# yahoo/bftkv

Measured on AMD Instinct MI355X. Metric: pgp_rsa2048_signature_verifies_per_sec, higher is better.
Workload: dtype u32; 1 GPU; 64-replica quorum, 10000 RSA-2048 signed writes per GPU (cfg2 of BASELINE.json), 534164 signature packets per GPU, 1.0% corrupt / 0.5% unknown issuer / 0.5% duplicate / 1.0% one-short; parallelism=shard-by-write x1, RCCL all-gather of verdict bitmaps on the verifier's stream, replicas=64, writes_per_gpu=10000, sigs_per_gpu=534164, batches_in_flight=3

## Files before the change

### bftkv_amd/csrc/capi.hip

```cpp
#include "../../include/bftkv_gpu.h"

#include <hip/hip_runtime.h>
#include <stdio.h>
#include <stdlib.h>
#include <string.h>

#include <limits.h>
#include <linux/futex.h>
#include <sched.h>
#include <sys/syscall.h>
#include <unistd.h>

#include <algorithm>
#include <array>
#include <atomic>
#include <memory>
#include <functional>
#include <map>
#include <set>
#include <chrono>
#include <condition_variable>
#include <mutex>
#include <shared_mutex>
#include <system_error>
// ... 28 lines not shown
  hipError_t ensure_exact(size_t bytes) {
    if (bytes <= cap) return hipSuccess;
    if (p) { hipError_t e = hipFree(p); if (e != hipSuccess) return e; p = nullptr; cap = 0; }
    hipError_t e = hipMalloc(&p, bytes);
    if (e == hipSuccess) cap = bytes;
    return e;
  }
  void release() { if (p) (void)hipFree(p); p = nullptr; cap = 0; }
  template <typename T> T* as() const { return (T*)p; }
};

struct KeyEntry {
  uint64_t key_id = 0, entity_id = 0;
  uint8_t algo = 0, flags = 0;
  uint32_t bits = 0, e = 0, n0 = 0, qbits = 0;
  std::vector<uint32_t> nl, r2, r2w, qw, dtab, qpow, qconst;
  std::string material;
  bool cert_only = false;
  int cert_group = -1;
  uint32_t entity_index = 0;
  std::string cert_digest;
  uint64_t last_used = 0;
  bool dsa_unslotted = false;
};

struct QuorumHost {
  bool live = false;
  int n_qcs = 0;
  int32_t f[MAX_QC], mn[MAX_QC], thr[MAX_QC], suff[MAX_QC];
  std::vector<std::vector<uint64_t>> nodes;
// ... 12 lines not shown
  hipStream_t stream = nullptr;
  hipStream_t stream_h = nullptr;
  hipStream_t stream_d = nullptr;
  std::recursive_mutex mu;
  std::string err;

  uint64_t keyring_gen = 0;
  uint32_t n_keys = 0, n_entities = 0;
  bool have_dsa_keys = false, have_rsa3072 = false, have_rsa4096 = false, have_ambiguous = false;
  std::vector<uint64_t> h_key_id, h_entity_id;
  std::vector<uint32_t> h_key_entity;
  std::vector<uint8_t> h_key_flags;
  std::vector<KeyEntry> ring, certs;
  uint32_t n_ring_entities = 0;
  std::map<std::string, bool> cert_valid;
  DevBuf k_r2w;
  DevBuf k_id, k_entity, k_algo, k_flags, k_bits, k_e, k_n, k_r2, k_n0, k_q, k_qbits, k_dsatab, k_dsaslot, k_sorted_id, k_sorted_slot;
  DevBuf dsa_comb;
  uint32_t dsa_wbits = 8, dsa_wbits_pinned = 0;
  std::map<std::string, uint32_t> dsa_comb_slot;
  std::set<std::string> dsa_cert_materials;
  uint64_t ring_epoch = 0, dsa_ring_epoch_seen = ~0ull;
  uint32_t dsa_wbits_want = 0;
  uint32_t dsa_entry_limbs = DSA_N_SMALL;
  size_t dsa_budget_bytes = 0;
  bool have_dsa3072 = false, have_dsa2048 = false;
  DevBuf dsa_idx;
  uint64_t cert_clock = 0;
  struct CertFast { uint64_t issuer_id; int group; uint64_t epoch; };
  std::shared_mutex cert_fast_mu;
  std::unordered_map<std::string, CertFast> cert_fast;
// ... 421 lines not shown
  if (total && !d_mid_in && plan_q && big && c->h_mail) {
    const auto t_spin = std::chrono::steady_clock::now();
    for (uint32_t it = 0;; ++it) {
      const uint32_t v = __atomic_load_n(&c->h_mail[3], __ATOMIC_ACQUIRE);
      if (v) { other_hashes = (v & 1u) != 0; break; }
      if ((it & 255u) == 255u && std::chrono::steady_clock::now() - t_spin > std::chrono::microseconds(300) + std::chrono::nanoseconds((uint64_t)total / 2)) break;
      __builtin_ia32_pause();
    }
  }
  if (total && !d_mid_in && other_hashes)
    hipLaunchKernelGGL(k_digest_other, dim3(std::min<uint32_t>((total + 255) / 256, DIGEST_OTHER_MAX_BLOCKS)), dim3(256), 0, s,
                       d_tbs, d_tbs_off, d_ss, c->mid.as<uint32_t>(), c->mid64.as<uint64_t>(), n_items, c->recs.as<SigRec>(), total,
                       c->digests.as<uint32_t>(), c->pk_count.as<uint32_t>() + 4, txt, n_recs_dev);
  const dim3 cg(((uint64_t)total * CMP_LANES + 255) / 256);
  auto launch_compare = [&](const uint32_t* start) {
    hipLaunchKernelGGL(k_rsa_compare, cg, dim3(256), 0, s, c->recs.as<SigRec>(), c->pk_list.as<uint32_t>(),
                       cnt_p, start, c->kt, c->r.as<uint32_t>(), c->digests.as<uint32_t>());
    if (c->have_rsa3072)
      hipLaunchKernelGGL(k_rsa_compare, cg, dim3(256), 0, s, c->recs.as<SigRec>(), c->pk_list3072.as<uint32_t>(),
                         cnt_p + 2, start + 2, c->kt, c->r3072.as<uint32_t>(), c->digests.as<uint32_t>());
    if (c->have_rsa4096)
      hipLaunchKernelGGL(k_rsa_compare, cg, dim3(256), 0, s, c->recs.as<SigRec>(), c->pk_list4096.as<uint32_t>(),
                         cnt_p + 3, start + 3, c->kt, c->r4096.as<uint32_t>(), c->digests.as<uint32_t>());
  };
  auto launch_dsa = [&](const uint32_t* start) {
    hipLaunchKernelGGL(k_dsa_mul, dim3((total + 63) / 64), dim3(64), 0, s, c->recs.as<SigRec>(), c->dsa_list.as<uint32_t>(),
                       cnt_p, start, c->kt, c->digests.as<uint32_t>(), c->dsa_u.as<uint32_t>());
    const uint32_t* idx_s = nullptr; const uint32_t* idx_b = nullptr; const uint32_t* cnt_cls = nullptr;
    if (c->have_dsa3072 && c->have_dsa2048) {
      uint32_t* cc = cnt_p + (start == start0 ? 20 : 22);
      uint32_t* is = c->dsa_idx.as<uint32_t>() + (start == start0 ? 0 : 2 * (size_t)total);
      hipLaunchKernelGGL(k_dsa_split, dim3((total + 255) / 256), dim3(256), 0, s, c->recs.as<SigRec>(), c->dsa_list.as<uint32_t>(), cnt_p, start, c->kt,
// ... 22 lines not shown
    pl.verdict = c->o_verdict.as<uint8_t>();
    hipLaunchKernelGGL(k_plan<2>, dim3((n_items + PLAN_ITEMS - 1) / PLAN_ITEMS), dim3(PLAN_BLOCK), 0, s, pl, c->kt, *plan_q);
    const uint32_t* const start1 = cnt_p + 8;
    if (c->have_dsa_keys) launch_dsa_inv(s, start1);
    launch_modexp(start1);
    launch_compare(start1);
    if (c->have_dsa_keys) launch_dsa(start1);
  }
  if (total && c->have_ambiguous && !d_msg_slot)
    hipLaunchKernelGGL(k_candidates, dim3((total + 63) / 64), dim3(64), 0, s, d_tbs, d_tbs_off, d_ss, d_mid_in ? d_mid_in : c->mid.as<uint32_t>(),
                       c->mid64.as<uint64_t>(), n_items, c->recs.as<SigRec>(), total, n_recs_dev, d_tbs_prefix, c->kt, d_cert_ent, d_sig_class, txt,
                       c->hash_mask.as<uint32_t>());
  HIPCHK(c, rec(3, s));
  HIPCHK(c, hipGetLastError());
  return 0;
}

int make_key_entry(bftkv_gpu_ctx* c, const bftkv_gpu_pubkey& k, bool cert_only, KeyEntry* out) {
  KeyEntry& e = *out;
  e.key_id = k.key_id; e.entity_id = k.entity_id; e.algo = k.pk_algo; e.cert_only = cert_only;
  e.material.clear();
  e.material.push_back((char)k.pk_algo);
  e.material.push_back((char)k.usable_sign);
  auto app = [&](const uint8_t* p, uint32_t l) {
    uint32_t z = 0;
    while (z < l && p[z] == 0) ++z;
    if (l > z) e.material.append((const char*)p + z, l - z);
    e.material.push_back('|');
  };
  app(k.n, k.n_len); app(k.e, k.e_len); app(k.g, k.g_len); app(k.y, k.y_len);
  e.flags = 0;
  if (k.usable_sign) e.flags |= KEYF_USABLE_SIGN;
  if (k.pk_algo != PK_RSA_ENCRYPT_ONLY && k.pk_algo != PK_ELGAMAL) e.flags |= KEYF_CAN_SIGN;
  if (k.key_id == k.entity_id) e.flags |= KEYF_PRIMARY;
  if (cert_only) e.flags |= KEYF_CERT_ONLY;
  e.bits = (uint32_t)hostbn::bit_length(k.n, k.n_len);
  e.e = 0; e.n0 = 0; e.qbits = 0;
  e.r2w.clear();
  e.nl.assign(MONT_NMAX, 0); e.r2.assign(MONT_NMAX, 0); e.qw.assign(8, 0); e.dtab.assign(2 * DSA_N_BIG, 0); e.qpow.clear(); e.qconst.clear();
  if (k.pk_algo == PK_RSA || k.pk_algo == PK_RSA_SIGN_ONLY) {
    if (hostbn::bit_length(k.e, k.e_len) > 32) return fail(c, BFTKV_E_UNSUPPORTED, "RSA public exponent wider than 32 bits");
    for (uint32_t j = 0; j < k.e_len; ++j) e.e = (e.e << 8) | k.e[j];
    const int nlimbs = e.bits <= 2048 ? MONT_N : (e.bits <= 3072 ? MONT_TPI_BIG * MONT_L3072 : MONT_TPI_BIG * MONT_L4096);
    if (e.bits > 4096) e.bits = 0xFFFFFFFFu;
    else if (!hostbn::mont_setup(k.n, k.n_len, nlimbs, e.nl.data(), e.r2.data(), &e.n0)) e.bits = 0xFFFFFFFFu;
    else if (e.bits <= 2048) {
      std::vector<uint32_t> nl80(80);
      uint32_t n0b = 0;
      e.r2w.assign(80, 0);
      (void)hostbn::mont_setup(k.n, k.n_len, 80, nl80.data(), e.r2w.data(), &n0b);
    }
  } else if (k.pk_algo == PK_DSA) {
    e.qbits = (uint32_t)hostbn::bit_length(k.e, k.e_len);
    const int NLp = e.bits <= 2048 ? (int)DSA_N_SMALL : (int)DSA_N_BIG;
    const uint32_t cap_bits = e.bits <= 2048 ? 2048u : 3072u;
    const int nwords = (28 * NLp + 31) / 32 + 1;
    std::vector<uint32_t> p(nwords), g(nwords), y(nwords), q(nwords);
    hostbn::from_be(k.e, k.e_len, q.data(), nwords);
    bool ok = e.bits >= 2 && e.bits <= 3072 && e.qbits >= 32 && e.qbits <= 256 && (q[0] & 1u) &&
              hostbn::mont_setup(k.n, k.n_len, NLp, e.nl.data(), e.r2.data(), &e.n0);
    if (ok && (hostbn::bit_length(k.g, k.g_len) > cap_bits || hostbn::bit_length(k.y, k.y_len) > cap_bits)) ok = false;
    if (ok) {
      hostbn::from_be(k.n, k.n_len, p.data(), nwords);
      hostbn::from_be(k.g, k.g_len, g.data(), nwords);
      hostbn::from_be(k.y, k.y_len, y.data(), nwords);
// ... 187 lines not shown
                         (uint32_t)cs.size(), d_slots.as<uint32_t>(), d_rows.as<uint32_t>(), c->kt, c->dsa_comb.as<uint32_t>(), parts);
    else
      hipLaunchKernelGGL((k_dsa_build_comb<MONT_L, MONT_TPI>), dim3((n_groups + QUADS_PER_BLOCK - 1) / QUADS_PER_BLOCK), dim3(RSA_BLOCK), 0, c->stream,
                         (uint32_t)cs.size(), d_slots.as<uint32_t>(), d_rows.as<uint32_t>(), c->kt, c->dsa_comb.as<uint32_t>(), parts);
    e = hipStreamSynchronize(c->stream);
    d_slots.release(); d_rows.release();
  }
  if (e != hipSuccess) return fail(c, BFTKV_E_DEVICE, "k_dsa_build_comb", e);
  return 0;
}

int upload_key_table(bftkv_gpu_ctx* c) {
  if (c->root) return fail(c, BFTKV_E_STATE, "a forked context cannot change the key table (use its root)");
  KtWrite kw(c);
  std::vector<uint64_t> key_id, entity_ids;
  std::vector<uint32_t> entity, bits, e32, nl, r2, r2w, n0, qw, qbits, dtab;
  std::vector<uint8_t> algo, flags;
  std::vector<const KeyEntry*> rows;
  auto add = [&](const KeyEntry& e, bool own_entity) {
    uint32_t ent = 0;
    if (own_entity) { ent = (uint32_t)entity_ids.size(); entity_ids.push_back(e.entity_id); }
    else {
      for (; ent < entity_ids.size(); ++ent) if (entity_ids[ent] == e.entity_id) break;
      if (ent == entity_ids.size()) entity_ids.push_back(e.entity_id);
    }
    key_id.push_back(e.key_id); entity.push_back(ent); algo.push_back(e.algo); flags.push_back(e.flags);
    bits.push_back(e.bits); e32.push_back(e.e); n0.push_back(e.n0); qbits.push_back(e.qbits);
    nl.insert(nl.end(), e.nl.begin(), e.nl.end()); r2.insert(r2.end(), e.r2.begin(), e.r2.end());
    r2w.insert(r2w.end(), e.r2w.begin(), e.r2w.end()); r2w.resize(key_id.size() * 80, 0);
    qw.insert(qw.end(), e.qw.begin(), e.qw.end()); dtab.insert(dtab.end(), e.dtab.begin(), e.dtab.end());
    rows.push_back(&e);
    return ent;
  };
  for (auto& e : c->ring) add(e, false);
  c->n_ring_entities = (uint32_t)entity_ids.size();
  int last_group = -1;
  uint32_t group_ent = 0;
  std::vector<uint32_t> group_ents;
  for (auto& e : c->certs) {
    if (e.cert_group != last_group) { group_ent = add(e, true); last_group = e.cert_group; }
    else {
      key_id.push_back(e.key_id); entity.push_back(group_ent); algo.push_back(e.algo); flags.push_back(e.flags);
      bits.push_back(e.bits); e32.push_back(e.e); n0.push_back(e.n0); qbits.push_back(e.qbits);
      nl.insert(nl.end(), e.nl.begin(), e.nl.end()); r2.insert(r2.end(), e.r2.begin(), e.r2.end());
      r2w.insert(r2w.end(), e.r2w.begin(), e.r2w.end()); r2w.resize(key_id.size() * 80, 0);
      qw.insert(qw.end(), e.qw.begin(), e.qw.end()); dtab.insert(dtab.end(), e.dtab.begin(), e.dtab.end());
      rows.push_back(&e);
    }
    const_cast<KeyEntry&>(e).entity_index = group_ent;
    if (e.cert_group >= 0) {
      if (group_ents.size() <= (size_t)e.cert_group) group_ents.resize((size_t)e.cert_group + 1, 0xFFFFFFFEu);
      group_ents[(size_t)e.cert_group] = group_ent;
    }
  }
  std::vector<uint32_t> sorted_slot(key_id.size());
  for (size_t i = 0; i < sorted_slot.size(); ++i) sorted_slot[i] = (uint32_t)i;
  std::stable_sort(sorted_slot.begin(), sorted_slot.end(), [&](uint32_t a, uint32_t b) { return key_id[a] < key_id[b]; });
  std::vector<uint64_t> sorted_id(key_id.size());
  for (size_t i = 0; i < sorted_slot.size(); ++i) sorted_id[i] = key_id[sorted_slot[i]];
  int rc;
  if ((rc = upload(c, c->k_sorted_id, sorted_id)) || (rc = upload(c, c->k_sorted_slot, sorted_slot))) return rc;
  if ((rc = upload(c, c->k_id, key_id)) || (rc = upload(c, c->k_entity, entity)) || (rc = upload(c, c->k_algo, algo)) ||
      (rc = upload(c, c->k_flags, flags)) || (rc = upload(c, c->k_bits, bits)) || (rc = upload(c, c->k_e, e32)) ||
      (rc = upload(c, c->k_n, nl)) || (rc = upload(c, c->k_r2, r2)) || (rc = upload(c, c->k_n0, n0)) ||
      (rc = upload(c, c->k_q, qw)) || (rc = upload(c, c->k_qbits, qbits)) || (rc = upload(c, c->k_dsatab, dtab)) || (rc = upload(c, c->k_r2w, r2w)))
    return rc;
  c->kt.r2_limbs80 = c->k_r2w.as<uint32_t>();
  c->n_keys = (uint32_t)key_id.size();
  c->kt.n_keys = c->n_keys;
  c->kt.n_limbs = c->k_n.as<uint32_t>();
  c->kt.r2_limbs = c->k_r2.as<uint32_t>();
  c->kt.n0inv = c->k_n0.as<uint32_t>();
  c->kt.dsa_tab = c->k_dsatab.as<uint32_t>();
  bool bits_changed = false;
  if ((rc = sync_dsa_tables(c, rows, algo, bits, &bits_changed))) return rc;
  if (bits_changed && (rc = upload(c, c->k_bits, bits))) return rc;
  HIPCHK(c, hipStreamSynchronize(c->stream));
  c->have_dsa_keys = c->have_dsa3072 = c->have_dsa2048 = c->have_rsa3072 = c->have_rsa4096 = c->have_ambiguous = false;
  for (size_t i = 0; i < algo.size(); ++i) {
    if (flags[i] & KEYF_AMBIGUOUS) c->have_ambiguous = true;
    if (algo[i] == PK_DSA) c->have_dsa_keys = true;
    if (algo[i] == PK_DSA && bits[i] != 0xFFFFFFFFu && bits[i] > 2048) c->have_dsa3072 = true;
// ... 122 lines not shown
  if (!c) return;
  for (bftkv_gpu_ctx* w : c->hb_workers) bftkv_gpu_destroy(w);
  c->hb_workers.clear();
  if (!c->root && c->n_forks.load() > 0) {
    fprintf(stderr, "bftkv_gpu_destroy: context still has %d forked context(s); not destroyed\n", c->n_forks.load());
    return;
  }
  {
    std::lock_guard<std::mutex> lk(g_live_mu);
    for (size_t i = 0; i < g_live.size(); ++i) if (g_live[i] == c) { g_live.erase(g_live.begin() + i); break; }
  }
  (void)hipSetDevice(c->device);
  (void)hipStreamSynchronize(c->stream);
  (void)hipStreamSynchronize(c->stream_h);
  (void)hipStreamSynchronize(c->stream_d);
  for (DevBuf* b : {&c->k_id, &c->k_entity, &c->k_algo, &c->k_flags, &c->k_bits, &c->k_e, &c->k_n, &c->k_r2, &c->k_n0, &c->k_q, &c->k_qbits, &c->k_dsatab, &c->k_dsaslot, &c->dsa_comb, &c->k_sorted_id, &c->k_sorted_slot, &c->k_r2w,
                    &c->chunk_arena, &c->chunk_ctr, &c->counts, &c->base, &c->total, &c->item_flags, &c->walk_scratch, &c->cert_ent, &c->sig_class, &c->mid, &c->mid64, &c->hash_mask, &c->recs, &c->digests, &c->r, &c->xr,
                    &c->pk_list, &c->pk_list3072, &c->pk_list4096, &c->r3072, &c->r4096, &c->pk_count, &c->dsa_list, &c->dsa_u, &c->dsa_idx, &c->ids_tmp, &c->o_err, &c->o_nver, &c->o_verdict, &c->o_fenced, &c->in_tbs, &c->in_tbs_off,
                    &c->in_ss, &c->in_ss_off, &c->in_prefix, &c->in_prefix_off, &c->in_shared, &c->in_shared_off, &c->in_seg, &c->st_tmp, &c->item_tmp, &c->bits_tmp, &c->plan_cut, &c->txt_mid32, &c->txt_mid64, &c->txt_tail, &c->txt_len})
    b->release();
  for (auto& q : c->quorums) { q.member.release(); q.ids.release(); }
  c->in_pack.release();
  c->forced_iss.release();
  release_small_pin(c);
  if (c->h_out) (void)hipHostFree(c->h_out);
  if (c->root) c->root->n_forks.fetch_sub(1);
  for (DevBuf* b : c->scratch_pool) { b->release(); delete b; }
  for (auto& kv : c->modtab_cache) for (DevBuf& b : kv.second) b.release();
  for (DevBuf& b : c->ec_fb_tab) b.release();
  if (c->h_mail) (void)hipHostFree(c->h_mail);
  if (c->hb_out) (void)hipHostFree(c->hb_out);
// ... 953 lines not shown
```

### bftkv_amd/csrc/device_types.h

```cpp
#pragma once
#include <stdint.h>

namespace bftkv {

enum SigStatus : uint8_t {
  ST_OK = 0,
  ST_UNKNOWN_ISSUER = 1,
  ST_PARSE_ERROR = 2,
  ST_NOT_SIGNATURE = 3,
  ST_NO_ISSUER = 4,
  ST_HASH_UNSUPPORTED = 5,
  ST_HASH_TAG = 6,
  ST_ALGO_MISMATCH = 7,
  ST_BAD_SIG = 8,
  ST_KEY_CANNOT_SIGN = 9,
  ST_UNSUPPORTED = 10,
  ST_NOT_EXAMINED = 11,
  ST_PENDING_CHUNKED = 98,
  ST_PENDING_PARSE = 99,
  ST_PENDING_HASH = 100,
  ST_PENDING_RSA = 101,
  ST_PENDING_DSA = 102,
};

// ... 21 lines not shown

struct KeyTableDev {
  uint32_t n_keys;
  const uint64_t* key_id;
  const uint64_t* sorted_id;
  const uint32_t* sorted_slot;
  const uint32_t* entity;
  const uint8_t* pk_algo;
  const uint8_t* flags;
  const uint32_t* mod_bits;
  const uint32_t* rsa_e;
  const uint32_t* n_limbs;
  const uint32_t* r2_limbs;
  const uint32_t* r2_limbs80;
  const uint32_t* n0inv;
  const uint32_t* q_words;
  const uint32_t* q_bits;
  const uint32_t* dsa_tab;
  const uint32_t* dsa_slot;
  const uint32_t* dsa_comb;
  uint32_t dsa_wbits;
  uint32_t dsa_entry_limbs;
  uint32_t hash_policy;
};
constexpr uint32_t dsa_nwin(uint32_t wbits) { return (256u + wbits - 1u) / wbits; }
constexpr uint32_t DSA_N_SMALL = 76, DSA_N_BIG = 112;
constexpr uint64_t dsa_comb_limbs_per_key(uint32_t wbits, uint32_t entry_limbs) {
  return 2ull * dsa_nwin(wbits) * ((1u << wbits) - 1u) * entry_limbs;
}
constexpr uint32_t dsa_qpow_words(uint32_t entry_limbs) { return entry_limbs * 10u; }
constexpr uint32_t dsa_qtail_words(uint32_t entry_limbs) { return dsa_qpow_words(entry_limbs) + 12u; }
constexpr bool dsa_plain_window(uint32_t base, uint32_t w, uint32_t nwin) { return base == 1u && w == nwin - 1u; }
constexpr uint64_t dsa_slot_stride(uint32_t wbits, uint32_t entry_limbs) { return dsa_comb_limbs_per_key(wbits, entry_limbs) + dsa_qtail_words(entry_limbs); }

constexpr uint8_t KEYF_USABLE_SIGN = 1, KEYF_CAN_SIGN = 2, KEYF_PRIMARY = 4;
constexpr uint8_t KEYF_CERT_ONLY = 8;
constexpr uint8_t KEYF_CERT_CHECK_ONLY = 16;
constexpr uint8_t KEYF_AMBIGUOUS = 32;
constexpr uint32_t ITEM_FENCED = 0x80000000u;
constexpr uint32_t ITEM_TEXT_SHIFT = 8, ITEM_NEEDS_PAYLOAD = 0x7F7Eu;

struct TextDev {
  uint32_t* mid32;
  uint64_t* mid64;
  uint8_t* tail;
  uint64_t* len;
};

// ... 12 lines not shown
```

### bftkv_amd/csrc/host_bignum.h

```cpp
#pragma once
#include <stdint.h>
#include <string.h>

#include <vector>

namespace bftkv {
namespace hostbn {

constexpr int W28 = 28;
constexpr uint32_t MASK28 = (1u << W28) - 1;

inline void from_be(const uint8_t* be, uint32_t len, uint32_t* w, int nwords) {
  memset(w, 0, sizeof(uint32_t) * nwords);
  for (uint32_t i = 0; i < len; ++i) {
    uint32_t k = len - 1 - i;
    if ((int)(k >> 2) < nwords) w[k >> 2] |= (uint32_t)be[i] << (8 * (k & 3));
  }
}

inline int bit_length(const uint8_t* be, uint32_t len) {
  uint32_t i = 0;
  while (i < len && be[i] == 0) ++i;
  if (i == len) return 0;
  int top = 8;
// ... 120 lines not shown
  const uint32_t e = 2u * 28u * (uint32_t)nlimbs;
  int hb = 31;
  while (!((e >> hb) & 1u)) --hb;
  for (int b = hb - 1; b >= 0; --b) {
    montmul64(acc.data(), acc.data(), m.data(), m0inv, k, acc.data());
    if ((e >> b) & 1u) dbl_mod64(acc.data(), m.data(), k);
  }
  one[0] = 1;
  montmul64(acc.data(), one.data(), m.data(), m0inv, k, acc.data());
  std::vector<uint32_t> r(nwords, 0);
  for (int i = 0; i < nwords && i < 2 * k; ++i) r[i] = (uint32_t)(acc[i >> 1] >> (32 * (i & 1)));
  to_limbs28(r.data(), nwords, r2_limbs, nlimbs);
  return true;
}

inline void add_mod(uint32_t* a, const uint32_t* b, const uint32_t* m, int n) {
  uint64_t c = 0;
  for (int i = 0; i < n; ++i) { c += (uint64_t)a[i] + b[i]; a[i] = (uint32_t)c; c >>= 32; }
  if (c || cmp(a, m, n) >= 0) sub(a, m, n);
}
inline void mul_mod(const uint32_t* a, const uint32_t* b, const uint32_t* m, uint32_t* r, int n) {
  std::vector<uint32_t> acc(n, 0);
  for (int i = 32 * n - 1; i >= 0; --i) {
    dbl_mod(acc.data(), m, n);
    if ((b[i >> 5] >> (i & 31)) & 1u) add_mod(acc.data(), a, m, n);
  }
  memcpy(r, acc.data(), sizeof(uint32_t) * n);
}
inline void reduce(uint32_t* a, const uint32_t* m, int n) {
  std::vector<uint32_t> r(n, 0);
// ... 19 lines not shown
```

### bftkv_amd/csrc/kernels.hip

```cpp
#include <hip/hip_runtime.h>
#include <stdint.h>

#include "device_types.h"
#include "mont28.h"
#include "u256.h"
#include "hashes.h"

namespace bftkv {

struct ParsedPacket {
  uint64_t next;
  bool event;
  SigRec rec;
};

__host__ __device__ __forceinline__ bool known_tag(uint32_t tag) {
  return tag < 32 && ((0x00066BFEu >> tag) & 1u);
}

struct SubpacketState {
  bool have_ctime = false, have_issuer = false, have_embedded = false;
  bool too_deep = false;
  uint64_t issuer = 0;
};
// ... 1117 lines not shown
__device__ __forceinline__ uint32_t em_head_limb(uint32_t gi, uint32_t kbytes) {
  const int32_t top = 8 * ((int32_t)kbytes - 2), lo = (int32_t)gi * MONT_W;
  if (top < lo) return 0u;
  if (top >= lo + MONT_W - 1) return MONT_MASK;
  return (1u << (top - lo + 1)) - 1u;
}

template <int L, int TPI>
__global__ void __launch_bounds__(MODEXP_BLOCK, 3) k_rsa_modexp(const uint8_t* __restrict__ sig_blob, const SigRec* __restrict__ recs,
                                                          const uint32_t* __restrict__ pk_list, const uint32_t* __restrict__ pk_count_ptr,
                                                          const uint32_t* __restrict__ pk_start_ptr,
                                                          KeyTableDev kt, uint32_t* __restrict__ r_low,
                                                          uint32_t* __restrict__ xr_scratch, uint64_t* __restrict__ clk) {
  constexpr int NL = TPI * L;
  constexpr int GROUPS = MODEXP_BLOCK / TPI;
  const bool stamp = clk && blockIdx.x == 0 && threadIdx.x == 0;
  uint64_t t0 = 0, r0 = 0;
  if (stamp) { t0 = __builtin_readcyclecounter(); r0 = __builtin_amdgcn_s_memrealtime(); }
  __shared__ uint32_t a_sh[GROUPS * NL];
  __shared__ uint32_t x_sh[GROUPS * NL];
  const uint32_t count = *pk_count_ptr, start = *pk_start_ptr;
  if (start + blockIdx.x * GROUPS >= count) return;
  const uint32_t quad = threadIdx.x / TPI;
  const int qlane = threadIdx.x % TPI;
  const uint32_t gq = start + blockIdx.x * GROUPS + quad;
  const bool active = gq < count;
  const uint32_t pi = active ? gq : (count - 1);
  const uint32_t ri = pk_list[pi];
  const SigRec rec = recs[ri];
  const uint32_t key = (uint32_t)rec.key_slot;
// ... 17 lines not shown
  }
  const uint32_t n0inv = kt.n0inv[key];
  const uint32_t e = kt.rsa_e[key];
  const uint32_t kbytes = (kt.mod_bits[key] + 7) >> 3;
  const uint32_t cls = (e << 1) | (((e & 1u) && e > 1u && !(rec.flags & 1u)) ? 1u : 0u);

  uint64_t todo = __builtin_amdgcn_ballot_w64(true);
  while (todo) {
    const int lead = __builtin_ctzll(todo);
    const uint32_t cls_u = (uint32_t)__builtin_amdgcn_readlane((int)cls, lead);
    const bool live = (cls == cls_u);
    const uint32_t e_u = cls_u >> 1;
    const bool sc_u = cls_u & 1u;
    const int top = 31 - __builtin_clz(e_u | 1u);
    int kind = OP_TO_MONT, bitpos = top;
    while (true) {
      if (kind == OP_TO_MONT) {
#pragma unroll
        for (int k = 0; k < L; ++k) { b[k] = rp[k]; a_lds[k] = x_lds[k]; }
      } else {
#pragma unroll
        for (int k = 0; k < L; ++k) b[k] = y[k];
        if (kind == OP_SQR) {
#pragma unroll
          for (int k = 0; k < L; ++k) a_lds[k] = y[k];
        } else if (kind == OP_MULX) {
#pragma unroll
          for (int k = 0; k < L; ++k) a_lds[k] = xrp[k];
        } else if (kind == OP_MULP) {
#pragma unroll
          for (int k = 0; k < L; ++k) a_lds[k] = x_lds[k];
        } else {
#pragma unroll
          for (int k = 0; k < L; ++k) a_lds[k] = (qlane == 0 && k == 0) ? 1u : 0u;
        }
      }
      __builtin_amdgcn_fence(__ATOMIC_ACQ_REL, "wavefront");
      if (kind == OP_SQR) mont_mul<L, TPI, true>(y, a_rd, b, n, n0inv, qlane);
      else mont_mul<L, TPI, false>(y, a_rd, b, n, n0inv, qlane);
      __builtin_amdgcn_fence(__ATOMIC_ACQ_REL, "wavefront");
      if (kind == OP_TO_MONT && (e_u & (e_u - 1u)) != 0 && !(sc_u && __builtin_popcount(e_u) == 2)) {
#pragma unroll
        for (int k = 0; k < L; ++k) xrp[k] = y[k];
      }
      if (kind == OP_MULP || kind == OP_MUL1) break;
      if (kind == OP_SQR && ((e_u >> bitpos) & 1u)) { kind = (bitpos == 0 && sc_u) ? OP_MULP : OP_MULX; continue; }
      --bitpos;
      kind = (bitpos >= 0) ? OP_SQR : OP_MUL1;
    }
    canonicalize<L, TPI>(y, qlane);
    if (e_u == 0) {
#pragma unroll
      for (int k = 0; k < L; ++k) y[k] = (qlane == 0 && k == 0) ? 1u : 0u;
    }
    uint32_t head = 0;
#pragma unroll
    for (int k = 0; k < L; ++k) {
      const uint32_t gi = (uint32_t)qlane * L + k;
      if (gi >= (uint32_t)EM_LOW_LIMBS) head |= y[k] ^ em_head_limb(gi, kbytes);
    }
    head = grp_or<TPI>(head);
    if (head != 0 && qlane == 0) y[0] = EM_HEAD_BAD;
#pragma unroll
    for (int k = 0; k < L; ++k) a_lds[k] = y[k];
    __builtin_amdgcn_fence(__ATOMIC_ACQ_REL, "wavefront");
    if (live && active && qlane < 4) {
      uint32_t* out = r_low + (uint64_t)pi * EM_LOW_LIMBS + qlane * (EM_LOW_LIMBS / 4);
      const uint32_t* src = a_rd + qlane * (EM_LOW_LIMBS / 4);
// ... 74 lines not shown
  {
    const uint32_t n_valid = min((uint32_t)GROUPS, count - q0) * EM_LOW_LIMBS;
    const uint32_t* src = r_low + (uint64_t)q0 * EM_LOW_LIMBS;
    for (uint32_t t = threadIdx.x; t < GROUPS * EM_LOW_LIMBS; t += 256) r_sh[t] = t < n_valid ? src[t] : 0u;
    __syncthreads();
  }
  const uint32_t* rp = r_sh + (threadIdx.x / CMP_LANES) * EM_LOW_LIMBS + qlane * CMP_L;
  uint32_t diff = 0;
#pragma unroll
  for (int k = 0; k < CMP_L; ++k) {
    const int bit = MONT_W * k, wi = bit >> 5, sh = bit & 31;
    const uint32_t em = (sh == 0 ? Wn[wi] : __builtin_amdgcn_alignbit(Wn[wi + 1], Wn[wi], sh)) & MONT_MASK;
    diff |= em ^ rp[k];
  }
  diff = quad_or(diff);
  if (active && pending && qlane == 0) recs[ri].status = (diff == 0) ? ST_OK : ST_BAD_SIG;
}

constexpr int DSA_U_WORDS = 24;
__device__ __forceinline__ const uint32_t* dsa_slot_base(const KeyTableDev& kt, uint32_t key) {
  return kt.dsa_comb + (uint64_t)kt.dsa_slot[key] * dsa_slot_stride(kt.dsa_wbits, kt.dsa_entry_limbs);
}
__device__ __forceinline__ const uint32_t* dsa_qconst(const KeyTableDev& kt, uint32_t key) {
  return dsa_slot_base(kt, key) + dsa_comb_limbs_per_key(kt.dsa_wbits, kt.dsa_entry_limbs) + dsa_qpow_words(kt.dsa_entry_limbs);
}
__global__ void __launch_bounds__(64) k_dsa_inv(const uint8_t* __restrict__ sig_blob, const SigRec* __restrict__ recs,
                                                const uint32_t* __restrict__ dsa_list, const uint32_t* __restrict__ pk_count,
                                                const uint32_t* __restrict__ pk_start,
                                                KeyTableDev kt, uint32_t* __restrict__ dsa_u , uint32_t batch_min) {
  if (pk_count[1] - pk_start[1] >= batch_min) return;
// ... 742 lines not shown
```

### bftkv_amd/csrc/mont28.h

```cpp
#pragma once
#include <hip/hip_runtime.h>
#include <stdint.h>

namespace bftkv {

constexpr int MONT_W = 28;
constexpr uint32_t MONT_MASK = (1u << MONT_W) - 1;
constexpr int MONT_TPI = 4;
constexpr int MONT_L = 19;
constexpr int MONT_N = MONT_TPI * MONT_L;
constexpr int MONT_TPI_BIG = 8;
constexpr int MONT_L3072 = 14, MONT_L4096 = 19;
constexpr int MONT_NMAX = MONT_TPI_BIG * MONT_L4096;

constexpr int DPP_QUAD_BCAST0 = 0x00;
constexpr int DPP_QUAD_SHR1 = 0x90;
constexpr int DPP_QUAD_SWAP1 = 0xB1;
constexpr int DPP_QUAD_SWAP2 = 0x4E;
constexpr int DPP_ROW_SHL1 = 0x101;

__device__ __forceinline__ uint32_t dpp_quad_bcast0(uint32_t v) {
  return (uint32_t)__builtin_amdgcn_update_dpp(0, (int)v, DPP_QUAD_BCAST0, 0xF, 0xF, true);
}
__device__ __forceinline__ uint32_t dpp_quad_shr1(uint32_t v) {
// ... 26 lines not shown
__device__ __forceinline__ uint32_t grp_shr1(uint32_t v) {
  if constexpr (TPI == 4) return dpp_quad_shr1(v);
  else return dpp_row_shr1(v);
}
template <int TPI>
__device__ __forceinline__ uint32_t grp_or(uint32_t v) {
  v = quad_or(v);
  if constexpr (TPI == 8) v |= (uint32_t)__shfl_xor((int)v, 4);
  return v;
}

__device__ __forceinline__ uint64_t mad64(uint32_t a, uint32_t b, uint64_t c) {
  return (uint64_t)a * (uint64_t)b + c;
}

template <int L, int TPI = MONT_TPI, bool SQR = false>
__device__ __forceinline__ void mont_mul(uint32_t (&out)[L], const uint32_t* a_lds,
                                         const uint32_t (&b)[L], const uint32_t (&n)[L],
                                         uint32_t n0inv, int qlane) {
  constexpr bool NORM = 2 * TPI * L > 255;
  uint32_t mask_v;
  asm("v_mov_b32 %0, 0xfffffff" : "=v"(mask_v));
  uint64_t Q[2 * L - 1];
#pragma unroll
  for (int k = 0; k < L + (NORM ? 1 : 0); ++k) Q[k] = 0;

#pragma unroll 1
  for (int blk = 0; blk < TPI; ++blk) {
    const uint32_t* ap = a_lds + blk * L;
#pragma unroll
    for (int r = 0; r < L; ++r) {
      const uint32_t ai = ap[r];
      const uint32_t ai2 = ai << 1;
#pragma unroll
      for (int k = SQR ? r : 0; k < L; ++k) {
        const uint32_t av = (SQR && k > r) ? ai2 : ai;
        if (k == L - 1 && r > 0) Q[r + k] = mad64(av, b[k], (NORM && r == 1) ? Q[r + k] : 0);
        else Q[r + k] = mad64(av, b[k], Q[r + k]);
      }
      const uint32_t m = grp_bcast0<TPI>((uint32_t)Q[r] * n0inv, qlane) & mask_v;
#pragma unroll
      for (int k = 0; k < L; ++k) Q[r + k] = mad64(m, n[k], Q[r + k]);
      Q[r + 1] += Q[r] >> MONT_W;
// ... 84 lines not shown
```

Baseline: 148.5 million verifies/s.

## Verify RSA signatures by comparing Montgomery-domain result against precomputed EMSA frame constants

The modexp now starts directly from the signature in Montgomery form and skips the from-Montgomery conversion and the final multiply, writing the raw Montgomery-domain result to scratch. A new compare kernel reconstructs the expected value as digest*B + T[hash] using per-key constants precomputed on the host (EMSA-PKCS1 frame and scaling by R^-(e-1)). Because the digest occupies only one block of limbs, this needs a single partial Montgomery block. The aim is to cut the final conversion multiply and the exponentiation setup work per signature. In exchange it adds per-key host precomputation, a larger key table, and more complex correctness logic.

```diff
diff --git a/bftkv_amd/csrc/capi.hip b/bftkv_amd/csrc/capi.hip
--- a/bftkv_amd/csrc/capi.hip
+++ b/bftkv_amd/csrc/capi.hip
@@ -66,6 +66,7 @@
   uint64_t key_id = 0, entity_id = 0;
   uint8_t algo = 0, flags = 0;
   uint32_t bits = 0, e = 0, n0 = 0, qbits = 0;
+  std::vector<uint32_t> cmpk;
   std::vector<uint32_t> nl, r2, r2w, qw, dtab, qpow, qconst;
   std::string material;
   bool cert_only = false;
@@ -108,7 +109,7 @@
   std::vector<KeyEntry> ring, certs;
   uint32_t n_ring_entities = 0;
   std::map<std::string, bool> cert_valid;
-  DevBuf k_r2w;
+  DevBuf k_r2w, k_cmp;
   DevBuf k_id, k_entity, k_algo, k_flags, k_bits, k_e, k_n, k_r2, k_n0, k_q, k_qbits, k_dsatab, k_dsaslot, k_sorted_id, k_sorted_slot;
   DevBuf dsa_comb;
   uint32_t dsa_wbits = 8, dsa_wbits_pinned = 0;
@@ -560,8 +561,12 @@
                        c->digests.as<uint32_t>(), c->pk_count.as<uint32_t>() + 4, txt, n_recs_dev);
   const dim3 cg(((uint64_t)total * CMP_LANES + 255) / 256);
   auto launch_compare = [&](const uint32_t* start) {
+    if (wide8)
     hipLaunchKernelGGL(k_rsa_compare, cg, dim3(256), 0, s, c->recs.as<SigRec>(), c->pk_list.as<uint32_t>(),
                        cnt_p, start, c->kt, c->r.as<uint32_t>(), c->digests.as<uint32_t>());
+    else
+    hipLaunchKernelGGL(k_rsa_compare_full, cg, dim3(256), 0, s, c->recs.as<SigRec>(), c->pk_list.as<uint32_t>(),
+                       cnt_p, start, c->kt, c->xr.as<uint32_t>(), c->digests.as<uint32_t>());
     if (c->have_rsa3072)
       hipLaunchKernelGGL(k_rsa_compare, cg, dim3(256), 0, s, c->recs.as<SigRec>(), c->pk_list3072.as<uint32_t>(),
                          cnt_p + 2, start + 2, c->kt, c->r3072.as<uint32_t>(), c->digests.as<uint32_t>());
@@ -614,6 +619,27 @@
   HIPCHK(c, rec(3, s));
   HIPCHK(c, hipGetLastError());
   return 0;
+}
+
+static void emsa_frame_words(uint32_t kbytes, int idx, uint32_t* w, int nwords) {
+  static const uint8_t di_sha1[15] = {0x30, 0x21, 0x30, 0x09, 0x06, 0x05, 0x2b, 0x0e, 0x03, 0x02, 0x1a, 0x05, 0x00, 0x04, 0x14};
+  static const uint8_t di_sha2[19] = {0x30, 0x31, 0x30, 0x0d, 0x06, 0x09, 0x60, 0x86, 0x48, 0x01, 0x65, 0x03, 0x04, 0x02, 0x01, 0x05, 0x00, 0x04, 0x20};
+  static const uint8_t di_md5[18] = {0x30, 0x20, 0x30, 0x0c, 0x06, 0x08, 0x2a, 0x86, 0x48, 0x86, 0xf7, 0x0d, 0x02, 0x05, 0x05, 0x00, 0x04, 0x10};
+  static const uint8_t di_rmd160[14] = {0x30, 0x20, 0x30, 0x08, 0x06, 0x06, 0x28, 0xcf, 0x06, 0x03, 0x00, 0x31, 0x04, 0x14};
+  static const uint32_t dlen[N_HASHES] = {32, 28, 20, 64, 48, 16, 20}, plen[N_HASHES] = {19, 19, 15, 19, 19, 18, 14};
+  static const uint8_t sha2_arc[N_HASHES] = {1, 4, 0, 3, 2, 0, 0};
+  memset(w, 0, sizeof(uint32_t) * nwords);
+  const uint32_t hl = dlen[idx], pl = plen[idx], tl = hl + pl;
+  if (kbytes < tl + 11 || (int)((kbytes + 3) / 4) > nwords) return;
+  uint8_t pre[19];
+  if (idx == 2) memcpy(pre, di_sha1, pl);
+  else if (idx == 5) memcpy(pre, di_md5, pl);
+  else if (idx == 6) memcpy(pre, di_rmd160, pl);
+  else { memcpy(pre, di_sha2, pl); pre[1] = (uint8_t)(0x11 + hl); pre[14] = sha2_arc[idx]; pre[18] = (uint8_t)hl; }
+  auto set = [&](uint32_t i, uint32_t b) { w[i >> 2] |= b << (8 * (i & 3)); };
+  for (uint32_t i = 0; i < pl; ++i) set(hl + i, pre[pl - 1 - i]);
+  for (uint32_t i = tl + 1; i + 2 < kbytes; ++i) set(i, 0xFF);
+  set(kbytes - 2, 1);
 }
 
 int make_key_entry(bftkv_gpu_ctx* c, const bftkv_gpu_pubkey& k, bool cert_only, KeyEntry* out) {
@@ -636,7 +662,7 @@
   if (cert_only) e.flags |= KEYF_CERT_ONLY;
   e.bits = (uint32_t)hostbn::bit_length(k.n, k.n_len);
   e.e = 0; e.n0 = 0; e.qbits = 0;
-  e.r2w.clear();
+  e.r2w.clear(); e.cmpk.clear();
   e.nl.assign(MONT_NMAX, 0); e.r2.assign(MONT_NMAX, 0); e.qw.assign(8, 0); e.dtab.assign(2 * DSA_N_BIG, 0); e.qpow.clear(); e.qconst.clear();
   if (k.pk_algo == PK_RSA || k.pk_algo == PK_RSA_SIGN_ONLY) {
     if (hostbn::bit_length(k.e, k.e_len) > 32) return fail(c, BFTKV_E_UNSUPPORTED, "RSA public exponent wider than 32 bits");
@@ -649,6 +675,11 @@
       uint32_t n0b = 0;
       e.r2w.assign(80, 0);
       (void)hostbn::mont_setup(k.n, k.n_len, 80, nl80.data(), e.r2w.data(), &n0b);
+      constexpr int TW = 2048 / 32;
+      std::vector<uint32_t> frames((size_t)N_HASHES * TW);
+      for (int h = 0; h < N_HASHES; ++h) emsa_frame_words((e.bits + 7) >> 3, h, &frames[(size_t)h * TW], TW);
+      e.cmpk.assign(RSA_CMP_WORDS, 0);
+      if (!hostbn::rsa_cmp_constants(k.n, k.n_len, e.e, MONT_N, MONT_L, frames.data(), N_HASHES, TW, e.cmpk.data())) e.cmpk.clear();
     }
   } else if (k.pk_algo == PK_DSA) {
     e.qbits = (uint32_t)hostbn::bit_length(k.e, k.e_len);
@@ -866,7 +897,7 @@
   if (c->root) return fail(c, BFTKV_E_STATE, "a forked context cannot change the key table (use its root)");
   KtWrite kw(c);
   std::vector<uint64_t> key_id, entity_ids;
-  std::vector<uint32_t> entity, bits, e32, nl, r2, r2w, n0, qw, qbits, dtab;
+  std::vector<uint32_t> entity, bits, e32, nl, r2, r2w, n0, qw, qbits, dtab, cmpk;
   std::vector<uint8_t> algo, flags;
   std::vector<const KeyEntry*> rows;
   auto add = [&](const KeyEntry& e, bool own_entity) {
@@ -880,6 +911,7 @@
     bits.push_back(e.bits); e32.push_back(e.e); n0.push_back(e.n0); qbits.push_back(e.qbits);
     nl.insert(nl.end(), e.nl.begin(), e.nl.end()); r2.insert(r2.end(), e.r2.begin(), e.r2.end());
     r2w.insert(r2w.end(), e.r2w.begin(), e.r2w.end()); r2w.resize(key_id.size() * 80, 0);
+    cmpk.insert(cmpk.end(), e.cmpk.begin(), e.cmpk.end()); cmpk.resize(key_id.size() * RSA_CMP_WORDS, 0);
     qw.insert(qw.end(), e.qw.begin(), e.qw.end()); dtab.insert(dtab.end(), e.dtab.begin(), e.dtab.end());
     rows.push_back(&e);
     return ent;
@@ -896,6 +928,7 @@
       bits.push_back(e.bits); e32.push_back(e.e); n0.push_back(e.n0); qbits.push_back(e.qbits);
       nl.insert(nl.end(), e.nl.begin(), e.nl.end()); r2.insert(r2.end(), e.r2.begin(), e.r2.end());
       r2w.insert(r2w.end(), e.r2w.begin(), e.r2w.end()); r2w.resize(key_id.size() * 80, 0);
+      cmpk.insert(cmpk.end(), e.cmpk.begin(), e.cmpk.end()); cmpk.resize(key_id.size() * RSA_CMP_WORDS, 0);
       qw.insert(qw.end(), e.qw.begin(), e.qw.end()); dtab.insert(dtab.end(), e.dtab.begin(), e.dtab.end());
       rows.push_back(&e);
     }
@@ -915,9 +948,11 @@
   if ((rc = upload(c, c->k_id, key_id)) || (rc = upload(c, c->k_entity, entity)) || (rc = upload(c, c->k_algo, algo)) ||
       (rc = upload(c, c->k_flags, flags)) || (rc = upload(c, c->k_bits, bits)) || (rc = upload(c, c->k_e, e32)) ||
       (rc = upload(c, c->k_n, nl)) || (rc = upload(c, c->k_r2, r2)) || (rc = upload(c, c->k_n0, n0)) ||
-      (rc = upload(c, c->k_q, qw)) || (rc = upload(c, c->k_qbits, qbits)) || (rc = upload(c, c->k_dsatab, dtab)) || (rc = upload(c, c->k_r2w, r2w)))
+      (rc = upload(c, c->k_q, qw)) || (rc = upload(c, c->k_qbits, qbits)) || (rc = upload(c, c->k_dsatab, dtab)) || (rc = upload(c, c->k_r2w, r2w)) ||
+      (rc = upload(c, c->k_cmp, cmpk)))
     return rc;
   c->kt.r2_limbs80 = c->k_r2w.as<uint32_t>();
+  c->kt.rsa_cmp = c->k_cmp.as<uint32_t>();
   c->n_keys = (uint32_t)key_id.size();
   c->kt.n_keys = c->n_keys;
   c->kt.n_limbs = c->k_n.as<uint32_t>();
@@ -1070,7 +1105,7 @@
   (void)hipStreamSynchronize(c->stream);
   (void)hipStreamSynchronize(c->stream_h);
   (void)hipStreamSynchronize(c->stream_d);
-  for (DevBuf* b : {&c->k_id, &c->k_entity, &c->k_algo, &c->k_flags, &c->k_bits, &c->k_e, &c->k_n, &c->k_r2, &c->k_n0, &c->k_q, &c->k_qbits, &c->k_dsatab, &c->k_dsaslot, &c->dsa_comb, &c->k_sorted_id, &c->k_sorted_slot, &c->k_r2w,
+  for (DevBuf* b : {&c->k_id, &c->k_entity, &c->k_algo, &c->k_flags, &c->k_bits, &c->k_e, &c->k_n, &c->k_r2, &c->k_n0, &c->k_q, &c->k_qbits, &c->k_dsatab, &c->k_dsaslot, &c->dsa_comb, &c->k_sorted_id, &c->k_sorted_slot, &c->k_r2w, &c->k_cmp,
                     &c->chunk_arena, &c->chunk_ctr, &c->counts, &c->base, &c->total, &c->item_flags, &c->walk_scratch, &c->cert_ent, &c->sig_class, &c->mid, &c->mid64, &c->hash_mask, &c->recs, &c->digests, &c->r, &c->xr,
                     &c->pk_list, &c->pk_list3072, &c->pk_list4096, &c->r3072, &c->r4096, &c->pk_count, &c->dsa_list, &c->dsa_u, &c->dsa_idx, &c->ids_tmp, &c->o_err, &c->o_nver, &c->o_verdict, &c->o_fenced, &c->in_tbs, &c->in_tbs_off,
                     &c->in_ss, &c->in_ss_off, &c->in_prefix, &c->in_prefix_off, &c->in_shared, &c->in_shared_off, &c->in_seg, &c->st_tmp, &c->item_tmp, &c->bits_tmp, &c->plan_cut, &c->txt_mid32, &c->txt_mid64, &c->txt_tail, &c->txt_len})
diff --git a/bftkv_amd/csrc/device_types.h b/bftkv_amd/csrc/device_types.h
--- a/bftkv_amd/csrc/device_types.h
+++ b/bftkv_amd/csrc/device_types.h
@@ -59,6 +59,7 @@
   const uint32_t* r2_limbs;
   const uint32_t* r2_limbs80;
   const uint32_t* n0inv;
+  const uint32_t* rsa_cmp;
   const uint32_t* q_words;
   const uint32_t* q_bits;
   const uint32_t* dsa_tab;
@@ -77,6 +78,9 @@
 constexpr uint32_t dsa_qtail_words(uint32_t entry_limbs) { return dsa_qpow_words(entry_limbs) + 12u; }
 constexpr bool dsa_plain_window(uint32_t base, uint32_t w, uint32_t nwin) { return base == 1u && w == nwin - 1u; }
 constexpr uint64_t dsa_slot_stride(uint32_t wbits, uint32_t entry_limbs) { return dsa_comb_limbs_per_key(wbits, entry_limbs) + dsa_qtail_words(entry_limbs); }
+
+constexpr uint32_t RSA_CMP_ROWS = 8, RSA_CMP_LIMBS = 76;
+constexpr uint32_t RSA_CMP_WORDS = 2 * RSA_CMP_ROWS * RSA_CMP_LIMBS;
 
 constexpr uint8_t KEYF_USABLE_SIGN = 1, KEYF_CAN_SIGN = 2, KEYF_PRIMARY = 4;
 constexpr uint8_t KEYF_CERT_ONLY = 8;
diff --git a/bftkv_amd/csrc/host_bignum.h b/bftkv_amd/csrc/host_bignum.h
--- a/bftkv_amd/csrc/host_bignum.h
+++ b/bftkv_amd/csrc/host_bignum.h
@@ -158,6 +158,67 @@
   return true;
 }
 
+inline void halve_mod64(uint64_t* a, const uint64_t* m, int k) {
+  if (a[0] & 1) {
+    unsigned __int128 c = 0;
+    for (int i = 0; i < k; ++i) { c += (unsigned __int128)a[i] + m[i]; a[i] = (uint64_t)c; c >>= 64; }
+  }
+  for (int i = 0; i < k; ++i) a[i] = (a[i] >> 1) | (i + 1 < k ? a[i + 1] << 63 : 0);
+}
+
+inline bool rsa_cmp_constants(const uint8_t* n_be, uint32_t n_len, uint32_t e, int nlimbs, int blk_limbs, const uint32_t* t_words,
+                              int n_t, int t_nwords, uint32_t* out) {
+  const int bits = bit_length(n_be, n_len);
+  const size_t rows = (size_t)1 + n_t;
+  memset(out, 0, sizeof(uint32_t) * 2 * rows * nlimbs);
+  if (bits < 2 || !(n_be[n_len - 1] & 1)) return false;
+  const int k = (bits + 64) / 64;
+  const int nwords = 2 * k;
+  std::vector<uint32_t> nw(nwords);
+  from_be(n_be, n_len, nw.data(), nwords);
+  std::vector<uint64_t> m(k), bn(k, 0), g(k, 0), cm(k, 0), t(k), r(k);
+  for (int i = 0; i < k; ++i) m[i] = (uint64_t)nw[2 * i] | ((uint64_t)nw[2 * i + 1] << 32);
+  uint64_t m0inv = m[0];
+  for (int i = 0; i < 6; ++i) m0inv *= 2ull - m[0] * m0inv;
+  m0inv = 0ull - m0inv;
+  auto put = [&](const uint64_t* v, int path, size_t row) {
+    std::vector<uint32_t> w(nwords);
+    for (int i = 0; i < k; ++i) { w[2 * i] = (uint32_t)v[i]; w[2 * i + 1] = (uint32_t)(v[i] >> 32); }
+    to_limbs28(w.data(), nwords, out + ((size_t)path * rows + row) * nlimbs, nlimbs);
+  };
+  auto load_t = [&](int h) {
+    for (int i = 0; i < k; ++i) {
+      const uint32_t lo = 2 * i < t_nwords ? t_words[(size_t)h * t_nwords + 2 * i] : 0u;
+      const uint32_t hi = 2 * i + 1 < t_nwords ? t_words[(size_t)h * t_nwords + 2 * i + 1] : 0u;
+      t[i] = (uint64_t)lo | ((uint64_t)hi << 32);
+    }
+  };
+  bn[0] = 1;
+  for (int i = 0; i < 28 * blk_limbs; ++i) dbl_mod64(bn.data(), m.data(), k);
+  put(bn.data(), 0, 0);
+  for (int h = 0; h < n_t; ++h) { load_t(h); put(t.data(), 0, 1 + (size_t)h); }
+  if (!(e & 1u) || e <= 1u) return true;
+  g[0] = 1;
+  for (int i = 64 * k; i < 28 * nlimbs; ++i) halve_mod64(g.data(), m.data(), k);
+  for (int i = 28 * nlimbs; i < 64 * k; ++i) dbl_mod64(g.data(), m.data(), k);
+  const uint32_t x = e - 1u;
+  int hb = 31;
+  while (!((x >> hb) & 1u)) --hb;
+  cm = g;
+  for (int b = hb - 1; b >= 0; --b) {
+    montmul64(cm.data(), cm.data(), m.data(), m0inv, k, cm.data());
+    if ((x >> b) & 1u) montmul64(cm.data(), g.data(), m.data(), m0inv, k, cm.data());
+  }
+  montmul64(cm.data(), bn.data(), m.data(), m0inv, k, r.data());
+  put(r.data(), 1, 0);
+  for (int h = 0; h < n_t; ++h) {
+    load_t(h);
+    montmul64(cm.data(), t.data(), m.data(), m0inv, k, r.data());
+    put(r.data(), 1, 1 + (size_t)h);
+  }
+  return true;
+}
+
 inline void add_mod(uint32_t* a, const uint32_t* b, const uint32_t* m, int n) {
   uint64_t c = 0;
   for (int i = 0; i < n; ++i) { c += (uint64_t)a[i] + b[i]; a[i] = (uint32_t)c; c >>= 32; }
diff --git a/bftkv_amd/csrc/kernels.hip b/bftkv_amd/csrc/kernels.hip
--- a/bftkv_amd/csrc/kernels.hip
+++ b/bftkv_amd/csrc/kernels.hip
@@ -1155,6 +1155,7 @@
                                                           uint32_t* __restrict__ xr_scratch, uint64_t* __restrict__ clk) {
   constexpr int NL = TPI * L;
   constexpr int GROUPS = MODEXP_BLOCK / TPI;
+  constexpr bool PLAIN = (L == MONT_L && TPI == MONT_TPI);
   const bool stamp = clk && blockIdx.x == 0 && threadIdx.x == 0;
   uint64_t t0 = 0, r0 = 0;
   if (stamp) { t0 = __builtin_readcyclecounter(); r0 = __builtin_amdgcn_s_memrealtime(); }
@@ -1202,6 +1203,12 @@
     const bool sc_u = cls_u & 1u;
     const int top = 31 - __builtin_clz(e_u | 1u);
     int kind = OP_TO_MONT, bitpos = top;
+    const bool plain = PLAIN && sc_u;
+    if (plain) {
+#pragma unroll
+      for (int k = 0; k < L; ++k) y[k] = x_lds[k];
+      kind = OP_SQR; bitpos = top - 1;
+    }
     while (true) {
       if (kind == OP_TO_MONT) {
 #pragma unroll
@@ -1231,8 +1238,8 @@
 #pragma unroll
         for (int k = 0; k < L; ++k) xrp[k] = y[k];
       }
-      if (kind == OP_MULP || kind == OP_MUL1) break;
-      if (kind == OP_SQR && ((e_u >> bitpos) & 1u)) { kind = (bitpos == 0 && sc_u) ? OP_MULP : OP_MULX; continue; }
+      if (kind == OP_MUL1 || (kind == OP_MULP && bitpos == 0)) break;
+      if (kind == OP_SQR && ((e_u >> bitpos) & 1u)) { kind = (plain || (bitpos == 0 && sc_u)) ? OP_MULP : OP_MULX; continue; }
       --bitpos;
       kind = (bitpos >= 0) ? OP_SQR : OP_MUL1;
     }
@@ -1240,6 +1247,21 @@
     if (e_u == 0) {
 #pragma unroll
       for (int k = 0; k < L; ++k) y[k] = (qlane == 0 && k == 0) ? 1u : 0u;
+    }
+    if constexpr (PLAIN) {
+#pragma unroll
+      for (int k = 0; k < L; ++k) a_lds[k] = y[k];
+      __builtin_amdgcn_fence(__ATOMIC_ACQ_REL, "wavefront");
+      const uint64_t wr = __builtin_amdgcn_ballot_w64(live && active);
+      const uint32_t lane = threadIdx.x & 63u, wq0 = (threadIdx.x / 64u) * (64u / TPI);
+      const uint32_t* src = a_sh + wq0 * NL;
+      uint32_t* dst = xr_scratch + (uint64_t)(start + blockIdx.x * GROUPS + wq0) * NL;
+#pragma unroll 1
+      for (uint32_t j = lane; j < (uint32_t)(NL * (64 / TPI)); j += 64u)
+        if ((wr >> ((j / NL) * TPI)) & 1ull) dst[j] = src[j];
+      __builtin_amdgcn_fence(__ATOMIC_ACQ_REL, "wavefront");
+      todo &= ~__builtin_amdgcn_ballot_w64(live);
+      continue;
     }
     uint32_t head = 0;
 #pragma unroll
@@ -1344,6 +1366,58 @@
     diff |= em ^ rp[k];
   }
   diff = quad_or(diff);
+  if (active && pending && qlane == 0) recs[ri].status = (diff == 0) ? ST_OK : ST_BAD_SIG;
+}
+
+static_assert(RSA_CMP_ROWS == 1 + N_HASHES && RSA_CMP_LIMBS == MONT_N, "KeyTableDev::rsa_cmp layout");
+__global__ void __launch_bounds__(256) k_rsa_compare_full(SigRec* __restrict__ recs, const uint32_t* __restrict__ pk_list,
+                                                          const uint32_t* __restrict__ pk_count_ptr, const uint32_t* __restrict__ pk_start_ptr,
+                                                          KeyTableDev kt,
+                                                          const uint32_t* __restrict__ y_rows, const uint32_t* __restrict__ digests) {
+  constexpr int L = MONT_L, TPI = MONT_TPI, GROUPS = 256 / TPI;
+  const uint32_t count = *pk_count_ptr, start = *pk_start_ptr;
+  const uint32_t q0 = start + blockIdx.x * GROUPS;
+  if (q0 >= count) return;
+  const uint32_t gq = q0 + threadIdx.x / TPI;
+  const int qlane = threadIdx.x % TPI;
+  const bool active = gq < count;
+  const uint32_t pi = active ? gq : (count - 1);
+  const uint32_t ri = pk_list[pi];
+  const SigRec rec = recs[ri];
+  const bool pending = rec.status == ST_PENDING_RSA;
+  const uint32_t key = (uint32_t)rec.key_slot;
+  const uint32_t e = kt.rsa_e[key];
+  const uint32_t path = ((e & 1u) && e > 1u && !(rec.flags & 1u)) ? 1u : 0u;
+  const HashInfo hi = hash_info(rec.hash_id);
+  __shared__ uint32_t d_sh[GROUPS * L];
+  uint32_t* dl = d_sh + (threadIdx.x / TPI) * L;
+  const uint32_t* dgw = digests + (uint64_t)ri * 16;
+  const uint32_t hw = hi.dlen >> 2;
+  auto d_word = [&](uint32_t w) -> uint32_t { return w < hw ? __builtin_bswap32(dgw[hw - 1 - w]) : 0u; };
+  constexpr int DPL = (L + TPI - 1) / TPI;
+#pragma unroll
+  for (int t = 0; t < DPL; ++t) {
+    const uint32_t j = (uint32_t)qlane * DPL + t, bit = j * MONT_W, wi = bit >> 5, sh = bit & 31u;
+    if (j < (uint32_t)L) dl[j] = __builtin_amdgcn_alignbit(d_word(wi + 1), d_word(wi), sh) & MONT_MASK;
+  }
+  uint32_t n[L], b[L], w[L], y[L];
+  const uint32_t* np = kt.n_limbs + (uint64_t)key * MONT_NMAX + qlane * L;
+  const uint32_t* kp = kt.rsa_cmp + ((uint64_t)key * 2 + path) * (RSA_CMP_ROWS * RSA_CMP_LIMBS) + qlane * L;
+  const uint32_t* tp = kp + (1 + hi.idx) * RSA_CMP_LIMBS;
+  const uint32_t* yp = y_rows + (uint64_t)pi * MONT_N + qlane * L;
+#pragma unroll
+  for (int k = 0; k < L; ++k) { n[k] = np[k]; b[k] = kp[k]; }
+  __builtin_amdgcn_fence(__ATOMIC_ACQ_REL, "wavefront");
+  mont_mul<L, TPI, false, 1>(w, d_sh + (threadIdx.x / TPI) * L, b, n, kt.n0inv[key], qlane);
+#pragma unroll
+  for (int k = 0; k < L; ++k) { w[k] += tp[k]; y[k] = yp[k]; }
+  canonicalize<L, TPI>(w, qlane);
+  reduce_once<L, TPI>(w, n, qlane);
+  reduce_once<L, TPI>(y, n, qlane);
+  uint32_t diff = 0;
+#pragma unroll
+  for (int k = 0; k < L; ++k) diff |= w[k] ^ y[k];
+  diff = grp_or<TPI>(diff);
   if (active && pending && qlane == 0) recs[ri].status = (diff == 0) ? ST_OK : ST_BAD_SIG;
 }
 
diff --git a/bftkv_amd/csrc/mont28.h b/bftkv_amd/csrc/mont28.h
--- a/bftkv_amd/csrc/mont28.h
+++ b/bftkv_amd/csrc/mont28.h
@@ -64,7 +64,7 @@
   return (uint64_t)a * (uint64_t)b + c;
 }
 
-template <int L, int TPI = MONT_TPI, bool SQR = false>
+template <int L, int TPI = MONT_TPI, bool SQR = false, int NBLK = TPI>
 __device__ __forceinline__ void mont_mul(uint32_t (&out)[L], const uint32_t* a_lds,
                                          const uint32_t (&b)[L], const uint32_t (&n)[L],
                                          uint32_t n0inv, int qlane) {
@@ -76,7 +76,7 @@
   for (int k = 0; k < L + (NORM ? 1 : 0); ++k) Q[k] = 0;
 
 #pragma unroll 1
-  for (int blk = 0; blk < TPI; ++blk) {
+  for (int blk = 0; blk < NBLK; ++blk) {
     const uint32_t* ap = a_lds + blk * L;
 #pragma unroll
     for (int r = 0; r < L; ++r) {
```

Result: faster. 151.2 million verifies/s, median of 6 (+1.8%).
